# biiiipy/JaxMARL-HFT

Measured on AMD Instinct MI355X. Metric: env steps/sec (whole node), 2-agent MARL, 10-level LOB, NUM_ENVS=4096, higher is better.
Workload: dtype int32

## Files before the change

### jaxmarl-hft_amd/csrc/hftlob.hip

```cpp
#include <hip/hip_runtime.h>
#include <stdint.h>
#include <string.h>
#include <stdio.h>
#include <mutex>
#include <type_traits>
#include <limits.h>

#include "../../include/hftlob.h"

typedef int32_t i32;
typedef uint32_t u32;
typedef uint8_t u8;
#define DEV __device__ __forceinline__

DEV int lane_id() { return __lane_id(); }
DEV i32 rdl(i32 v, int l) { return __builtin_amdgcn_readlane(v, l); }
DEV i32 wrl(i32 old, i32 val, int l) { return __lane_id() == l ? val : old; }
DEV i32 uni(i32 v) { return __builtin_amdgcn_readfirstlane(v); }
DEV float unif(float v) { return __int_as_float(__builtin_amdgcn_readfirstlane(__float_as_int(v))); }
DEV i32 wadd(i32 a, i32 b) { return (i32)((u32)a + (u32)b); }
DEV i32 wsub(i32 a, i32 b) { return (i32)((u32)a - (u32)b); }
DEV i32 wmul(i32 a, i32 b) { return (i32)((u32)a * (u32)b); }
DEV i32 iabs_(i32 a) { return a < 0 ? wsub(0, a) : a; }
DEV i32 isign(i32 a) { return (a > 0) - (a < 0); }
// ... 1514 lines not shown
    i32* st = rec + c.off_agents;
    int ag = 0;
    for (int t = 0; t < nTy; ++t) {
        const hftlob_agent_type_cfg& tc = c.types[t];
        i32 sell = tc.task == HFTLOB_TASK_SELL ? 1 : 0;
        if (tc.kind == HFTLOB_AGENT_EXE && tc.task == HFTLOB_TASK_RANDOM)
            sell = randint(split_key(key, nTy + 1, t, part), 0, 2, part);
        for (int i = 0; i < tc.n_agents; ++i, ++ag) {
            i32 s[13];
            if (tc.kind == HFTLOB_AGENT_MM) {
                s[0] = 0; s[1] = 0; s[2] = 0; s[3] = fbit(0.0f); s[4] = fbit(0.0f);
            } else {
                s[0] = fbit(mid); s[1] = tc.task_size; s[2] = 0; s[3] = sell; s[4] = fbit(mid / (float)c.tick_size);
                for (int k = 5; k < 13; ++k) s[k] = fbit(0.0f);
            }
            const int nw = agent_words(tc);
            i32 v = 0;
            for (int k = 0; k < 13; ++k) if (l == k) v = s[k];
            if (l < nw) st[l] = v;
            if (obs) write_obs<false>(c, tc, wv, s, obs + (size_t)ag * c.obs_stride, false, ftime);
            st += nw;
        }
    }
}

template <int S>
__global__ __launch_bounds__(64) void k_env_reset(hftlob_env_cfg c, int n_env, const u32* __restrict__ keys,
                                                  const i32* __restrict__ init_states, i32* __restrict__ state,
                                                  float* __restrict__ obs) {
    one_wave();
    const int e = blockIdx.x;
    if (e >= n_env) return;
    Valid<S> VS, VT;
    VS.init(c.lob.n_orders);
    VT.init(c.lob.n_trades);
    Key k{keys[2 * e], keys[2 * e + 1]};
    env_reset_dev<S>(c, k, init_states, state + (size_t)e * c.rec_words,
                     obs ? obs + (size_t)e * c.n_agents * c.obs_stride : nullptr, VS, VT, c.ep_type == 1);
}

struct ActX {
    i32 bid_price, ask_price, bid_dist, ask_dist, bid_quant, ask_quant;
};

DEV void put_row(i32* lds_rows, int row, i32 f0, i32 f1, i32 f2, i32 f3, i32 f4, i32 f5, i32 f6, i32 f7) {
    const int l = lane_id();
    i32 v = f0;
    v = l == 1 ? f1 : v; v = l == 2 ? f2 : v; v = l == 3 ? f3 : v;
    v = l == 4 ? f4 : v; v = l == 5 ? f5 : v; v = l == 6 ? f6 : v; v = l == 7 ? f7 : v;
    if (l < 8) lds_rows[row * 8 + l] = v;
}

template <int S>
DEV void cancel_rows(const Side<S>& s, int R, const Valid<S>& V, i32 agent, int size, i32 side, i32 t, i32 tns,
                     i32* lds_rows, int row0) {
    int n = 0;
    i32 tid[S], q[S], o[S];
    const i32 (&p)[S] = s.pc;
    ldcol(s.t, R, FTID, tid);
    ldcol(s.t, R, FQ, q);
    ldcol(s.t, R, FOID, o);
#pragma unroll
    for (int r = 0; r < S; ++r) {
        lmask bm = V.m[r] & bal(tid[r] == agent);
        while (bm && n < size) {
            const int ln = (int)__builtin_ctzll(bm);
            bm &= bm - 1;
            put_row(lds_rows, row0 + n, 2, side, rdl(q[r], ln), rdl(p[r], ln), rdl(o[r], ln), agent, t, tns);
            ++n;
        }
    }
    for (; n < size; ++n) put_row(lds_rows, row0 + n, 2, side, 0, 0, 0, 0, t, tns);
}

template <int n>
DEV void filter_rows(i32* lds_rows, int arow, int crow, i32* scratch) {
    wave_sync();
    const int l = lane_id();
    const bool is_a = l < n, is_c = (l >= 8) & (l < 8 + n);
    const int row = is_a ? arow + l : (is_c ? crow + l - 8 : arow);
    const i32 p = lds_rows[row * 8 + 3], q = lds_rows[row * 8 + 2];
    lmask ma = 0, mc = 0;
#pragma unroll
    for (int k = 0; k < n; ++k) {
        const i32 cpk = rdl(p, 8 + k), apk = rdl(p, k);
        ma |= bal(is_a & (p != 0) & (p == cpk));
        mc |= bal(is_c & (apk != 0) & (p == apk));
    }
    constexpr lmask amask = (1ull << n) - 1, cmask = amask << 8;
    const int na = __builtin_popcountll(ma), nc = __builtin_popcountll(mc);
    const lmask mine = is_a ? ma : mc, all = is_a ? amask : cmask;
    const bool matched = (mine >> l) & 1ull;
    const lmask below = matched ? mine : (~mine & all);
    const int cnt = (int)__builtin_amdgcn_mbcnt_hi((u32)(below >> 32), __builtin_amdgcn_mbcnt_lo((u32)below, 0u));
    const int rank = matched ? cnt : (is_a ? na : nc) + cnt;
    if (l < 16) scratch[l] = 0;
    wave_sync();
    if ((is_a | is_c) & matched) scratch[(is_c ? 8 : 0) + rank] = q;
    wave_sync();
    const i32 av = scratch[rank & 7], cv = scratch[8 + (rank & 7)];
    const i32 nq = wsub(q, cv >= av ? av : 0);
    if (is_a & (nq == 0)) {
        reinterpret_cast<int4*>(lds_rows + row * 8)[0] = make_int4(0, 0, 0, 0);
        reinterpret_cast<int4*>(lds_rows + row * 8)[1] = make_int4(0, 0, 0, 0);
    } else if (is_a | is_c) {
        lds_rows[row * 8 + 2] = nq;
    }
    wave_sync();
}

template <int S>
DEV bool masked_best(const hftlob_env_cfg& c, Book<S>& B, i32 tid, i32 last_ba, i32 last_bb, i32& ba, i32& bb) {
    const i32 tick = c.tick_size;
    i32 mn = INT_MAX, mx = INT_MIN, at_[S], bt_[S];
    const i32 (&ap_)[S] = B.a.pc;
    const i32 (&bp_)[S] = B.b.pc;
    ldcol(B.a.t, B.c.nO, FTID, at_);
    ldcol(B.b.t, B.c.nO, FTID, bt_);
#pragma unroll
    for (int r = 0; r < S; ++r) {
        const i32 pa = (B.vs.v[r] && at_[r] != tid) ? ap_[r] : -1;
        const i32 pb = (B.vs.v[r] && bt_[r] != tid) ? bp_[r] : -1;
        mn = imin_(mn, B.vs.v[r] ? (pa == -1 ? c.lob.maxint : pa) : INT_MAX);
        mx = imax_(mx, B.vs.v[r] ? pb : INT_MIN);
    }
    ba = wave_min(mn);
    bb = wave_max(mx);
    ba = ba == c.lob.maxint ? -1 : ba;
    const bool empty = (ba == -1) || (bb == -1);
    ba = wmul(tick_floordiv(c, ba), tick);
    bb = wmul(tick_floordiv(c, bb), tick);
    if (empty) { bb = last_bb; ba = last_ba; }
    return empty;
}
template <int S>
DEV void mm_fixed_quant(const hftlob_env_cfg& c, const hftlob_agent_type_cfg& tc, Book<S>& B, const i32* st, i32 tid,
                        i32 action, i32 wt0, i32 wt1, i32 last_ba, i32 last_bb, i32* lds_rows, int row, ActX& x) {
    if (tc.fixed_action_setting) action = tc.fixed_action;
    const i32 tick = c.tick_size;
    i32 ba, bb;
    const bool empty = masked_best(c, B, tid, last_ba, last_bb, ba, bb);
    const float hsp = fmaxf(i2f(wsub(ba, bb)) / 2.0f, (float)tick / 2.0f);
    const float hs = (tick_ffloordiv(c, hsp) + 1.0f) * (float)tick;
    float bo, ao;
    i32 bq, aq;
    if (!tc.sell_buy_all_option) {
        const int ai = action < 0 ? imax_(action + 10, 0) : (action > 9 ? 9 : action);
        bo = (float)((0x0152043210ull >> (4 * ai)) & 0xF);
        ao = (float)((0x0510243210ull >> (4 * ai)) & 0xF);
        const i32 q1 = ai == 9 ? 0 : 1;
        bq = wmul(q1, tc.fixed_quant_value);
        aq = wmul(q1, tc.fixed_quant_value);
    } else {
        const int ai = action < 0 ? imax_(action + 9, 0) : (action > 8 ? 8 : action);
        const i32 bot[9] = {10, 2, 4, -1, 0, 2, -20, 0, 0}, aot[9] = {10, 2, 4, -1, 2, 0, 0, -20, 0};
        const i32 iq = ifloordiv(st[2], tc.fixed_quant_value);
        i32 b = bot[0], a = aot[0];
#pragma unroll
        for (int k = 1; k < 9; ++k) { b = ai == k ? bot[k] : b; a = ai == k ? aot[k] : a; }
        bo = i2f(b);
        ao = i2f(a);
        bq = wmul(ai < 6 ? 1 : (ai == 6 ? iq : 0), tc.fixed_quant_value);
        aq = wmul(ai < 6 ? 1 : (ai == 7 ? iq : 0), tc.fixed_quant_value);
    }
    if (empty) { bq = 0; aq = 0; }
    const float bpf = i2f(bb) - bo * hs;
    const float apf = i2f(ba) + ao * hs;
    const i32 bp = f2i(tick_ffloordiv(c, fmaxf(bpf, 0.0f)) * (float)tick);
    const i32 ap = f2i(tick_ffloordiv(c, fmaxf(i2f(wadd(bp, tick)), apf)) * (float)tick);
    i32 typ0 = 1, typ1 = 1, sd0 = 1, sd1 = -1, qq0 = bq, qq1 = aq, pp0 = bp, pp1 = ap;
    const i32 inv = st[2];
    const i32 lq0 = f2i(tc.auto_liquidate_alpha * i2f(imax_(wsub(0, inv), 0)));
    const i32 lq1 = f2i(tc.auto_liquidate_alpha * i2f(imax_(inv, 0)));
    const i32 lp0 = f2i(i2f(ba) + hs * 10.0f), lp1 = f2i(i2f(bb) - hs * 10.0f);
    const bool liq = (tc.tenth_action_market && action == 9) ||
                     (tc.auto_liquidate_threshold != 0 && iabs_(inv) > tc.auto_liquidate_threshold);
    if (liq) { typ0 = typ1 = 4; sd0 = -1; sd1 = 1; qq0 = lq0; qq1 = lq1; pp0 = lp0; pp1 = lp1; }
    const i32 ta = wadd(wt0, tc.time_delay_obs_act), tb = wadd(wt1, tc.time_delay_obs_act);
    put_row(lds_rows, row, typ0, sd0, qq0, pp0, c.placeholder_order_id, tid, ta, tb);
    put_row(lds_rows, row + 1, typ1, sd1, qq1, pp1, c.placeholder_order_id, tid, ta, tb);
    x.bid_price = bp; x.ask_price = ap; x.bid_dist = wsub(bb, bp); x.ask_dist = wsub(ap, ba);
    x.bid_quant = bq; x.ask_quant = aq;
}

DEV i32 f2i_sat(float f) {
    return f != f ? 0 : (f >= 2147483648.0f ? INT_MAX : (f <= -2147483648.0f ? INT_MIN : (i32)f));
}
template <int S>
DEV void mm_other_actions(const hftlob_env_cfg& c, const hftlob_agent_type_cfg& tc, Book<S>& B, const i32* st, i32 tid,
                          i32 action, i32 wt0, i32 wt1, i32 last_ba, i32 last_bb, i32 step, i32 init_t0, i32* lds_rows,
                          int row, ActX& x) {
    if (tc.fixed_action_setting) action = tc.fixed_action;
    const i32 tick = c.tick_size, inv = st[2], fq = tc.fixed_quant_value;
    const int kind = tc.action_space;
    const int na = kind == HFTLOB_MM_ACT_SIMPLE ? (tc.simple_nothing_action ? 4 : 3)
                                                 : (kind == HFTLOB_MM_ACT_AVST ? 8 : 2 * tc.bob_v0 + 1);
    int ai = action < 0 ? action + na : action;
    ai = ai < 0 ? 0 : (ai >= na ? na - 1 : ai);
    i32 bp, ap, bq, aq, bdist = 0, adist = 0, bpost = 0, apost = 0;
    if (kind == HFTLOB_MM_ACT_BOB_RL || kind == HFTLOB_MM_ACT_BOB_STRATEGY || kind == HFTLOB_MM_ACT_AVST) {
        i32 ba, bb;
        const bool empty = masked_best(c, B, tid, last_ba, last_bb, ba, bb);
        if (kind == HFTLOB_MM_ACT_BOB_RL) {
            const i32 v0 = tc.bob_v0, d = (ai & 1) ? (ai + 1) / 2 : -(ai / 2);
            bq = wmul(wadd(v0, d), fq);
            aq = wmul(wsub(v0, d), fq);
            if (empty) { bq = 0; aq = 0; }
            bp = bb; ap = ba;
        } else if (kind == HFTLOB_MM_ACT_BOB_STRATEGY) {
            const float kappa = i2f(wadd(action, 1)) / i2f(wmul(tc.bob_v0, 5));
            const float pos = i2f(inv), v0 = (float)tc.bob_v0;
            bq = f2i_sat(rintf(v0 * fmaxf(1.0f - kappa * pos, 0.0f)));
            aq = f2i_sat(rintf(v0 * fmaxf(1.0f + kappa * pos, 0.0f)));
            if (empty) { bq = 0; aq = 0; }
            bp = bb; ap = ba;
        } else {
            const i32 mid = ifloordiv(wadd(ba, bb), 2);
            const float gam[8] = {0.1f, 0.2f, 0.5f, 1.0f, 2.0f, 5.0f, 10.0f, 20.0f};
            float gamma = gam[0], lt = tc.avst_log_term[0];
#pragma unroll
            for (int k = 1; k < 8; ++k) if (ai == k) { gamma = gam[k]; lt = tc.avst_log_term[k]; }
            const i32 tl = c.ep_type == 1 ? wsub(c.episode_time, wsub(wt0, init_t0)) : wsub(c.episode_time, step);
            const float nt = i2f(tl) / i2f(c.episode_time);
            const float res = i2f(mid) - i2f(inv) * gamma * tc.avst_var * nt;
            float spread = gamma * tc.avst_var * nt + (2.0f / gamma) * lt;
            spread = fminf(fmaxf(spread, (float)tick), (float)c.lob.maxint);
            float bf = res - spread / 2.0f, af = res + spread / 2.0f;
            bf = fminf(fmaxf(bf, 0.0f), (float)c.lob.maxint);
            af = fminf(fmaxf(af, 0.0f), (float)c.lob.maxint);
            bp = f2i_sat(tick_ffloordiv(c, bf) * (float)tick);
            ap = f2i_sat(tick_ffloordiv(c, af) * (float)tick);
            const i32 q = tick_floordiv(c, mid), rm = wsub(mid, wmul(q, tick));
            bp = imin_(bp, wmul(wsub(q, rm == 0 ? 1 : 0), tick));
            ap = imax_(ap, wmul(wadd(q, 1), tick));
            bq = fq; aq = fq;
            bdist = wsub(bb, bp); adist = wsub(ap, ba); bpost = bp; apost = ap;
        }
    } else {
        const i32 ba = wmul(tick_floordiv(c, last_ba), tick), bb = wmul(tick_floordiv(c, last_bb), tick);
        if (kind == HFTLOB_MM_ACT_SPREAD_SKEW) {
            const float mid = i2f(wadd(ba, bb)) / 2.0f;
            const i32 cur = wsub(ba, bb);
            const i32 st_ = ifloordiv(action, 3), sk = wsub(action, wmul(st_, 3));
            const float mult = st_ == 0 ? 1.0f : tc.spread_multiplier;
            const float nsp = i2f(cur) * mult;
            const float skt = sk == 0 ? -tc.skew_multiplier : (sk == 1 ? 0.0f : tc.skew_multiplier);
            const float smid = mid + skt * (tc.multiplier_type ? nsp : (float)tick);
            const float hs = ffloordiv(nsp, 2.0f);
            bp = f2i_sat(tick_ffloordiv(c, smid - hs) * (float)tick);
            ap = f2i_sat(tick_ffloordiv(c, smid + hs) * (float)tick);
            bq = fq; aq = fq;
        } else {
            const float bo = ai == 1 ? -2000.0f : 0.0f, ao = ai == 2 ? -2000.0f : 0.0f;
            if (tc.sell_buy_all_option) {
                const i32 big = imax_(iabs_(inv), fq);
                const i32 bqa = inv > 0 ? fq : big, aqa = inv > 0 ? big : fq;
                bq = ai == 0 ? fq : (ai == 1 ? bqa : 0);
                aq = ai == 0 ? fq : (ai == 2 ? aqa : 0);
            } else {
                bq = wmul((ai == 0 || ai == 1) ? 1 : 0, fq);
                aq = wmul((ai == 0 || ai == 2) ? 1 : 0, fq);
            }
            const float to = (float)wmul(tc.n_ticks_offset, tick);
            const float bf = i2f(bb) - bo * to, af = i2f(ba) + ao * to;
            bp = f2i_sat(tick_ffloordiv(c, fmaxf(bf, 0.0f)) * (float)tick);
            ap = f2i_sat(tick_ffloordiv(c, af) * (float)tick);
        }
    }
    const i32 ta = wadd(wt0, tc.time_delay_obs_act), tb = wadd(wt1, tc.time_delay_obs_act);
    put_row(lds_rows, row, 1, 1, bq, bp, c.placeholder_order_id, tid, ta, tb);
    put_row(lds_rows, row + 1, 1, -1, aq, ap, c.placeholder_order_id, tid, ta, tb);
    x.bid_price = bpost; x.ask_price = apost; x.bid_dist = bdist; x.ask_dist = adist;
    x.bid_quant = bq; x.ask_quant = aq;
}

DEV void mm_directional(const hftlob_env_cfg& c, const hftlob_agent_type_cfg& tc, i32 tid, i32 action, i32 wt0, i32 wt1,
                        i32 last_ba, i32 last_bb, i32* lds_rows, int row, ActX& x) {
    const i32 tick = c.tick_size;
    const i32 ba = wmul(tick_floordiv(c, last_ba), tick), bb = wmul(tick_floordiv(c, last_bb), tick);
    const int ai = action < 0 ? imax_(action + 3, 0) : (action > 2 ? 2 : action);
    const i32 bq = (ai == 1) * tc.fixed_quant_value, aq = (ai == 2) * tc.fixed_quant_value;
    const i32 ta = wadd(wt0, tc.time_delay_obs_act), tb = wadd(wt1, tc.time_delay_obs_act);
    put_row(lds_rows, row, 1, 1, bq, ba, c.placeholder_order_id, tid, ta, tb);
    put_row(lds_rows, row + 1, 1, -1, aq, bb, c.placeholder_order_id, tid, ta, tb);
    x.bid_price = x.ask_price = x.bid_dist = x.ask_dist = 0;
    x.bid_quant = bq; x.ask_quant = aq;
}

DEV void exe_fqc(const hftlob_env_cfg& c, const hftlob_agent_type_cfg& tc, const i32* st, i32 tid, i32 action, i32 wt0,
                 i32 wt1, i32 last_ba, i32 last_bb, i32 step, i32 max_steps, i32* lds_rows, int row) {
    const i32 tick = c.tick_size;
    const i32 ba = wmul(tick_floordiv(c, last_ba), tick), bb = wmul(tick_floordiv(c, last_bb), tick);
    const i32 sell = st[3];
    i32 pl[4];
    if (sell) {
        pl[0] = bb;
        pl[1] = f2i(ceilf(tick_ffloordiv(c, i2f(wadd(bb, ba)) / 2.0f)) * (float)tick);
        pl[2] = ba;
        pl[3] = wadd(ba, wmul(tick, tc.n_ticks_in_book));
    } else {
        pl[0] = ba;
        pl[1] = wmul(tick_floordiv(c, ifloordiv(wadd(bb, ba), 2)), tick);
        pl[2] = bb;
        pl[3] = wsub(bb, wmul(tick, tc.n_ticks_in_book));
    }
    const i32 side = wsub(1, wmul(sell, 2));
    const i32 ta = wadd(wt0, tc.time_delay_obs_act), tb = wadd(wt1, tc.time_delay_obs_act);
    const i32 fq = tc.fixed_quant_value, left = wsub(st[1], st[2]);
    i32 q[4] = {0, 0, 0, 0};
    if (tc.action_space == HFTLOB_EXE_ACT_FIXED_QUANTS_COMPLEX) {
        const int ai = action < 0 ? imax_(action + 13, 0) : (action > 12 ? 12 : action);
        if (ai > 0) {
            const int lvl = (ai - 1) & 3, mul = (ai - 1) >> 2;
            const i32 v = wmul(mul == 0 ? 1 : (mul == 1 ? 2 : 5), fq);
#pragma unroll
            for (int k = 0; k < 4; ++k) q[k] = k == lvl ? v : 0;
        }
        const i32 tot = wadd(wadd(q[0], q[1]), wadd(q[2], q[3]));
        if (!(tot <= left)) { q[0] = f2i(floorf(i2f(left))); q[1] = q[2] = q[3] = 0; }
        for (int k = 0; k < 4; ++k) put_row(lds_rows, row + k, 1, side, q[k], pl[k], c.placeholder_order_id, tid, ta, tb);
        return;
    }
    if (tc.action_space == HFTLOB_EXE_ACT_FIXED_QUANTS_1MSG) {
        const int ai = action < 0 ? imax_(action + 5, 0) : (action > 4 ? 4 : action);
        i32 p = 0;
#pragma unroll
        for (int k = 0; k < 4; ++k) p = ai == k + 1 ? pl[k] : p;
        i32 qq = ai == 0 ? 0 : fq;
        qq = qq <= left ? qq : 0;
        put_row(lds_rows, row, 1, side, qq, p, c.placeholder_order_id, tid, ta, tb);
        return;
    }
    const i32 ft = sell ? bb : ba, nt = sell ? ba : bb;
    if (tc.action_space == HFTLOB_EXE_ACT_SIMPLEST_CASE) {
        const int ai = action < 0 ? imax_(action + 3, 0) : (action > 2 ? 2 : action);
        q[0] = ai == 1 ? fq : 0;
        q[1] = ai == 2 ? fq : 0;
        if (!(wadd(q[0], q[1]) <= left)) { q[0] = f2i(floorf(i2f(wmul(fq, left)))); q[1] = 0; }
    } else {
        const int ai = action < 0 ? imax_(action + 2, 0) : (action > 1 ? 1 : action);
        const i32 steps_left = wsub(wsub(max_steps, step), 1);
        const i32 qts = f2i_sat(ceilf(i2f(imax_(left, 0)) / i2f(steps_left)));
        q[0] = ai == 0 ? qts : 0;
        q[1] = ai == 1 ? qts : 0;
    }
    put_row(lds_rows, row, 1, side, q[0], ft, c.placeholder_order_id, tid, ta, tb);
    put_row(lds_rows, row + 1, 1, side, q[1], nt, c.placeholder_order_id, tid, ta, tb);
}

DEV void exe_fixed_prices(const hftlob_env_cfg& c, const hftlob_agent_type_cfg& tc, const i32* rec, const i32* st,
                          i32 tid, const i32 (&act)[4], i32 wt0, i32 wt1, i32* lds_rows, int row) {
    const i32 tick = c.tick_size, w = tc.n_actions, left = wsub(st[1], st[2]), sell = st[3];
    i32 sum = 0;
    for (int j = 0; j < w; ++j) sum = wadd(sum, act[j]);
    i32 q[4];
    const bool rescale = sum > left;
    for (int j = 0; j < 4; ++j) q[j] = rescale ? f2i_sat(i2f(act[j]) / i2f(sum) * i2f(left)) : act[j];
    const int M = c.n_msgs, m0 = M > 10 ? M - 10 : 0;
    float sa = 0.0f, sb = 0.0f;
    for (int m = m0; m < M; ++m) {
        sa += i2f(rec[c.off_best_asks + m * 2]);
        sb += i2f(rec[c.off_best_bids + m * 2]);
    }
    const float n = (float)(M - m0), ft = (float)tick;
    const i32 ba = f2i_sat(ffloordiv(sa / n, ft) * ft), bb = f2i_sat(ffloordiv(sb / n, ft) * ft);
    i32 lv[4];
    if (sell) {
        lv[0] = wmul(tick_floordiv(c, bb), tick);
        lv[1] = f2i_sat(ceilf(ffloordiv(i2f(wadd(bb, ba)) / 2.0f, ft)) * ft);
        lv[2] = ba;
        lv[3] = wadd(ba, wmul(tick, tc.n_ticks_in_book));
    } else {
        lv[0] = wmul(tick_floordiv(c, ba), tick);
        lv[1] = wmul(tick_floordiv(c, ifloordiv(wadd(bb, ba), 2)), tick);
        lv[2] = bb;
        lv[3] = wsub(bb, wmul(tick, tc.n_ticks_in_book));
    }
    i32 p[4];
    if (w == 4) { p[0] = lv[0]; p[1] = lv[1]; p[2] = lv[2]; p[3] = lv[3]; }
    else { p[0] = lv[0]; p[1] = lv[2]; p[2] = lv[3]; p[3] = 0; }
    if (w == 4 && lv[1] == lv[2]) {
        q[2] = wadd(q[2], q[1]);
        q[1] = 0;
        p[1] = -1;
    }
    const i32 side = wsub(1, wmul(sell, 2));
    const i32 ta = wadd(wt0, tc.time_delay_obs_act), tb = wadd(wt1, tc.time_delay_obs_act);
    for (int j = 0; j < w; ++j) put_row(lds_rows, row + j, 1, side, q[j], p[j], c.placeholder_order_id, tid, ta, tb);
}

template <int S>
struct TradeView {
    i32 P[S], Q[S], S4[S], PT[S], AT[S];
    bool valid[S];
};
template <int S>
DEV void trade_view(const Book<S>& B, TradeView<S>& V, bool use_ovr, int ovr_idx, const i32 (&ovr)[8]) {
    const int l = lane_id();
#pragma unroll
    for (int r = 0; r < S; ++r) {
        const bool o = use_ovr && (r * 64 + l == ovr_idx);
        const i32 p = o ? ovr[0] : B.tr.get(0, r), q = o ? ovr[1] : B.tr.get(1, r);
        const i32 s4 = o ? ovr[4] : B.tr.get(4, r), pt = o ? ovr[6] : B.tr.get(6, r), at = o ? ovr[7] : B.tr.get(7, r);
        const bool v = B.vt.v[r] && p >= 0;
// ... 739 lines not shown
    const StepKeys SK = batched ? load_keys(c, pre_keys) : step_keys<NFIX == 0>(c, key_n, ek, keys, master, mk);
    if (master && !batched) mk = SK.next_master;
    const Key key_reset = SK.key_reset;
    if (RC) {
        B.ek = c.shuffle_action_messages ? split_key(SK.k1, 2, 0, c.prng_partitionable) : SK.k1;
        B.nmsg = M;
        B.part = c.prng_partitionable;
    }
    SUBSTAMP(t_keys);
    const i32* Lr = rec + c.off_loaded;
    const i32* Wr = rec + c.off_world;
    const i32 ld_t0 = Lr[LD_T0], win = Lr[LD_WIN], max_steps = Lr[LD_MAXS], start_index = Lr[LD_START],
              step = Lr[LD_STEP];
    const i32 wt0 = Wr[W_T0], wt1 = Wr[W_T1], oidc = Wr[W_OIDC];
    const float wmid = bitf(Wr[W_MID]);
    const i32 old_last_ba = rec[c.off_best_asks + (M - 1) * 2], old_last_bb = rec[c.off_best_bids + (M - 1) * 2];
    bool excl_any = false, excl_cfg = false;
    for (int t = 0; t < c.n_types; ++t) {
        const bool ex = c.types[t].kind == HFTLOB_AGENT_MM && c.types[t].exclude_extreme_spreads;
        excl_cfg |= ex;
        if (emit && ex) {
            bool any = false;
            for (int m = l; m < M; m += 64) {
                const i32 pa = rec[c.off_best_asks + m * 2], pb = rec[c.off_best_bids + m * 2];
                any |= (i2f(wsub(pa, pb)) / (i2f(wadd(pa, pb)) / 2.0f)) > 0.1f;
            }
            excl_any = ballot(any) != 0ull;
        }
    }
    const bool store_best = NFIX == 0 || (!keep | excl_cfg);
    i32 dstart = wadd(start_index, wmul(D, step));
    dstart = imax_(0, imin_(dstart, c.n_data_rows - D));
    const bool ftime = NFIX == 0 && c.ep_type == 1;
    const i32 t_end = wadd(ld_t0, c.episode_time);
    int4 px = make_int4(0, 0, 0, 0), py = px;
    if ((l >= C + A) & (l < M)) {
        const i32* g = msg_data + (size_t)(dstart + l - (C + A)) * 8;
        ld_msg(g, px, py);
        if (ftime) fixed_time_mask(px, py, t_end);
    }
    if (resident) {
        relink_side(B.a, R, B.vs);
        relink_side(B.b, R, B.vs);
        B.fl = fl_carry | F_STALE_A | F_STALE_B | STALE_ANY;
    } else {
        B.fl = commit_side<true>(B.a, fa, R, B.vs) | commit_side<false>(B.b, fb, R, B.vs) | F_STALE_A | F_STALE_B | STALE_ANY;
        B.fl |= slow_bit(B.fl);
    }
    SUBSTAMP(t_load);

#ifdef HFTLOB_STAMPS
    unsigned long long acc_act = 0, acc_cnl = 0, acc_flt = 0, acc_mmr = 0, acc_exr = 0, acc_obs = 0;
#endif
    {
        int ag = 0, arow = C, crow = 0, aw = 0;
        const i32* st = rec + c.off_agents;
        for (int t = 0; t < c.n_types; ++t) {
            const hftlob_agent_type_cfg& tc = c.types[t];
            for (int i = 0; i < tc.n_agents; ++i, ++ag) {
                const i32 tid = wsub(tc.trader_id0, i);
                const int w = tc.action_width;
                i32* aio = actions_io ? actions_io + (size_t)e * c.action_words + aw : nullptr;
                aw += w;
                i32 act, av[4] = {0, 0, 0, 0};
                if (NFIX > 0 || w == 1) {
                    if (master) {
                        act = rdl(SK.acts, 32 + ag);
                        if (aio && l == 0) aio[0] = act;
                    } else {
                        act = aio[0];
                    }
                    av[0] = act;
                } else {
                    i32 v = 0;
                    if (master) {
                        const bool part = c.prng_partitionable;
                        const Key ka = split_key(split_key(SK.key, c.n_types, t, part), tc.n_agents, i, part);
                        v = randint_vec(ka, w, l < w ? l : 0, 0, action_hi(tc), part);
                        if (aio && l < w) aio[l] = v;
                    } else if (l < w) {
                        v = aio[l];
                    }
#pragma unroll
                    for (int j = 0; j < 4; ++j) av[j] = rdl(v, j);
                    act = av[0];
                }
                i32 s4[4];
                {
                    const int b = (int)(st - (rec + c.off_agents));
#pragma unroll
                    for (int k = 0; k < 4; ++k) s4[k] = agw_pre ? rdl(agw, b + k) : st[k];
                }
                ActX x{0, 0, 0, 0, 0, 0};
                SUBSTAMP(ta0);
#if defined(HFTLOB_KO_ACT) || defined(HFTLOB_KO_CNL)
                for (int k = 0; k < tc.n_msgs; ++k) {
#ifndef HFTLOB_KO_ACT
                    if (k < tc.n_action_msgs) continue;
#endif
#ifndef HFTLOB_KO_CNL
                    if (k >= tc.n_action_msgs) continue;
#endif
                    put_row(rows, k < tc.n_action_msgs ? arow + k : crow + k - tc.n_action_msgs, 0, 0, 0, 0, 0, 0, 0, 0);
                }
#endif
#ifdef HFTLOB_DUP_AGENT
                i32 z_ = 0;
                asm volatile("s_mov_b32 %0, 0" : "=s"(z_));
                for (int rep = 0; rep < 2; ++rep) {
                const i32 tid_r = tid ^ (rep * z_), act_r = act ^ (rep * z_), ba_r = old_last_ba ^ (rep * z_);
                const bool do_act = rep == 0 || (HFTLOB_DUP_AGENT & 1), do_cnl = rep == 0 || (HFTLOB_DUP_AGENT & 2);
#else
                {
                const i32 tid_r = tid, act_r = act, ba_r = old_last_ba;
                constexpr bool do_act = true, do_cnl = true;
#endif
                if (tc.kind == HFTLOB_AGENT_MM) {
#ifndef HFTLOB_KO_ACT
                    if (!do_act) {
                    } else if (tc.action_space == HFTLOB_MM_ACT_DIRECTIONAL)
                        mm_directional(c, tc, tid_r, act_r, wt0, wt1, ba_r, old_last_bb, rows, arow, x);
                    else if (tc.action_space == HFTLOB_MM_ACT_FIXED_QUANTS)
                        mm_fixed_quant(c, tc, B, s4, tid_r, act_r, wt0, wt1, ba_r, old_last_bb, rows, arow, x);
                    else
                        mm_other_actions(c, tc, B, s4, tid_r, act_r, wt0, wt1, ba_r, old_last_bb, step, ld_t0, rows,
                                         arow, x);
#endif
                    STAMP_ACC(acc_act, ta0);
                    SUBSTAMP(ta1);
                    const int sz = tc.n_msgs / 4;
#ifndef HFTLOB_KO_CNL
                    if (do_cnl) {
                        cancel_rows(B.b, R, B.vs, tid_r, sz, 1, wt0, wt1, rows, crow);
                        cancel_rows(B.a, R, B.vs, tid_r, sz, -1, wt0, wt1, rows, crow + sz);
                    }
#endif
                    STAMP_ACC(acc_cnl, ta1);
                } else {
#ifndef HFTLOB_KO_ACT
                    if (!do_act) {
                    } else if (NFIX == 0 && tc.action_space == HFTLOB_EXE_ACT_FIXED_PRICES)
                        exe_fixed_prices(c, tc, rec, s4, tid_r, av, wt0, wt1, rows, arow);
                    else
                        exe_fqc(c, tc, s4, tid_r, act_r, wt0, wt1, ba_r, old_last_bb, step, max_steps, rows, arow);
#endif
                    STAMP_ACC(acc_act, ta0);
                    SUBSTAMP(ta1);
#ifndef HFTLOB_KO_CNL
                    const i32 sell = s4[3];
                    if (do_cnl)
                        cancel_rows(sell ? B.a : B.b, R, B.vs, tid_r, tc.n_msgs / 2, wsub(1, wmul(sell, 2)), wt0, wt1,
                                    rows, crow);
#endif
                    STAMP_ACC(acc_cnl, ta1);
                }
                }
                SUBSTAMP(ta2);
                {
                    const i32 xv[6] = {x.bid_price, x.ask_price, x.bid_dist, x.ask_dist, x.bid_quant, x.ask_quant};
                    i32 v = 0;
#pragma unroll
                    for (int k = 0; k < 6; ++k) if (l == k) v = xv[k];
                    if (l < 6) axs[ag * 6 + l] = v;
                }
#ifndef HFTLOB_KO_FILTER
                if (tc.n_action_msgs == 2) filter_rows<2>(rows, arow, crow, B.a.scr);
                else if (tc.n_action_msgs == 4) filter_rows<4>(rows, arow, crow, B.a.scr);
                else if (NFIX == 0 && tc.n_action_msgs == 3) filter_rows<3>(rows, arow, crow, B.a.scr);
                else filter_rows<1>(rows, arow, crow, B.a.scr);
#endif
                STAMP_ACC(acc_flt, ta2);
                arow += tc.n_action_msgs;
                crow += tc.n_msgs - tc.n_action_msgs;
                st += agent_words(tc);
            }
        }
    }
    wave_sync();
    SUBSTAMP(t_rows);
    {
        i32 f[8];
        const bool act_lane = l < A;
        if (act_lane) {
#pragma unroll
            for (int k = 0; k < 8; ++k) f[k] = rows[(C + l) * 8 + k];
            f[4] = wsub(oidc, l);
        }
        int dest = l;
        if (c.shuffle_action_messages && A >= 2) {
            const u32 bits = SK.shuffle_bits;
            int rank = 0;
            for (int j = 0; j < A; ++j) {
                const u32 bj = (u32)rdl((i32)bits, j);
                rank += (bj < bits) || (bj == bits && j < l);
            }
            dest = rank;
        }
        wave_sync();
        if (act_lane) {
#pragma unroll
            for (int k = 0; k < 8; ++k) rows[(C + dest) * 8 + k] = f[k];
        }
        wave_sync();
    }

    STAMP(t_agents);
    if (!RA) trades_fill(B.tr, B.vt, -1);
    B.ntr = 0;
    const int AR = C + A;
    bool abort_any = false;
    i32 prev_a = -1, prev_b = -1;
    float mid_acc = 0.0f, pa_acc = 0.0f, pb_acc = 0.0f;
    i32 last_p_a = 0, last_p_b = 0, last_t0 = 0, last_t1 = 0;
    int4 nx = px, ny = py;
#ifndef HFTLOB_NO_CARRY
    i32* carry = B.filt - PAD_FILT + PAD_CARRY;
    if (!RA && resident) {
        const i32 v = carry[l & 15];
        B.a.best_p = rdl(v, 0); B.a.best_q = rdl(v, 1); B.a.xp = rdl(v, 2); B.a.top = rdl(v, 3);
        B.a.top_p = rdl(v, 4); B.a.top_ts = rdl(v, 5); B.a.top_tns = rdl(v, 6);
        B.b.best_p = rdl(v, 7); B.b.best_q = rdl(v, 8); B.b.top = rdl(v, 9); B.b.top_p = rdl(v, 10);
        B.b.top_ts = rdl(v, 11); B.b.top_tns = rdl(v, 12);
        B.fl &= ~(F_STALE_A | F_STALE_B | STALE_ANY);
    }
#endif
#ifdef HFTLOB_STAMPS_CHUNK
    unsigned long long acc_dec = 0, acc_pre = 0, acc_loop = 0, acc_post = 0;
#endif
    for (int base = 0; base < M; base += 64) {
#ifdef HFTLOB_STAMPS_CHUNK
        const unsigned long long tc0 = __builtin_amdgcn_s_memtime();
#endif
        const int row = base + l;
        int4 x = nx, y = ny;
        if (RA ? (base == 0) & (row < AR) : row < AR) {
            x = reinterpret_cast<const int4*>(rows + row * 8)[0];
            y = reinterpret_cast<const int4*>(rows + row * 8)[1];
        } else if (ftime && base > 0 && row >= AR) {
            fixed_time_mask(x, y, t_end);
        }
        if (msgs_out && row < M) {
            int4* mo = reinterpret_cast<int4*>(msgs_out + ((size_t)e * M + row) * 8);
            mo[0] = x;
            mo[1] = y;
        }
        {
            const bool nv = (row + 64 >= AR) & (row + 64 < M);
            ld_msg(msg_data + (size_t)(dstart + (nv ? row + 64 - AR : 0)) * 8, nx, ny);
        }
        if (RA && (base == 0)) {
            if (row + 64 < AR) {
                nx = reinterpret_cast<const int4*>(rows + (row + 64) * 8)[0];
                ny = reinterpret_cast<const int4*>(rows + (row + 64) * 8)[1];
            }
            wave_sync();
            trades_fill(B.tr, B.vt, -1);
        }
        decode_msgs(B.c, x, y);
        i32 rpa = 0, rqa = 0, rpb = 0, rqb = 0;
        const int cnt = uni(imin_(64, M - base));
#ifdef HFTLOB_STAMPS_CHUNK
        acc_dec += __builtin_amdgcn_s_memtime() - tc0;
#endif
        run_chunk<RC>(B, x, y, cnt, base, rpa, rqa, rpb, rqb CHUNK_ARGS);
#ifdef HFTLOB_STAMPS_CHUNK
        const unsigned long long tc1 = __builtin_amdgcn_s_memtime();
#endif
        abort_any |= bal((l < cnt) & ((rpa == -1) | (rpb == -1))) != 0ull;
        i32 pa = rpa, pb = rpb;
        if ((base == 0) & (l == 0)) {
            pa = pa == -1 ? old_last_ba : pa;
            pb = pb == -1 ? old_last_bb : pb;
        }
        const i32 caq = rpa == -1 ? 0 : rqa, cbq = rpb == -1 ? 0 : rqb;
        const i32 cap = ffill(pa, prev_a), cbp = ffill(pb, prev_b);
        prev_a = rdl(cap, cnt - 1);
        prev_b = rdl(cbp, cnt - 1);
        if ((row < M) & (store_best | (row == M - 1))) {
            reinterpret_cast<int2*>(rec + c.off_best_asks)[row] = make_int2(cap, caq);
            reinterpret_cast<int2*>(rec + c.off_best_bids)[row] = make_int2(cbp, cbq);
        }
        if (row < M) {
            const float mf = i2f(wadd(cbp, cap)) / 2.0f;
            mid_acc = base == 0 ? mf : mid_acc + mf;
            if (info_out) {
                pa_acc = base == 0 ? i2f(cap) : pa_acc + i2f(cap);
                pb_acc = base == 0 ? i2f(cbp) : pb_acc + i2f(cbp);
            }
// ... 643 lines not shown
                return fail(HFTLOB_EINVAL, "EXE action_width");
            if (tc.n_action_msgs != na || tc.n_msgs != 2 * na) return fail(HFTLOB_EINVAL, "EXE message counts");
            if (a == HFTLOB_EXE_ACT_TWAP && c->ep_type != 0) return fail(HFTLOB_EINVAL, "twap needs fixed_steps");
            if (tc.observation_space < 0 || tc.observation_space > HFTLOB_EXE_OBS_SIMPLEST_CASE)
                return fail(HFTLOB_EINVAL, "EXE observation_space");
        } else return fail(HFTLOB_EINVAL, "unknown agent kind");
    }
    if (agents != c->n_agents) return fail(HFTLOB_EINVAL, "n_agents mismatch");
    int words = 0;
    for (int t = 0; t < c->n_types; ++t) words += c->types[t].n_agents * c->types[t].action_width;
    if (words != c->action_words) return fail(HFTLOB_EINVAL, "action_words mismatch");
    return HFTLOB_OK;
}

static hftlob_env_cfg kernel_cfg(const hftlob_env_cfg* cfg) {
    hftlob_env_cfg c = *cfg;
    const uint32_t d = (uint32_t)c.tick_size;
    const int l = d > 1u ? 32 - __builtin_clz(d - 1u) : 0;
    c.tick_magic = (uint32_t)((((unsigned __int128)1 << (31 + l)) + d - 1u) / d);
    return c;
}

int hftlob_env_reset(const hftlob_env_cfg* cfg, int n_env, const uint32_t* keys, const int32_t* msg_data,
                     const int32_t* init_states, int32_t* state, const hftlob_step_out* out, void* stream) {
    int rc = check_env(cfg);
    if (rc) return rc;
    (void)msg_data;
    if (n_env < 0) return fail(HFTLOB_ESHAPE, "negative n_env");
    if (n_env == 0) return HFTLOB_OK;
    if (!keys || !init_states || !state) return fail(HFTLOB_ENULL, "null array");
    float* obs = out ? out->obs : nullptr;
    const int S = slot_sets(cfg->lob.n_orders > cfg->lob.n_trades ? cfg->lob.n_orders : cfg->lob.n_trades);
    hipStream_t st = (hipStream_t)stream;
    dim3 g(n_env), b(ENV_BLOCK);
    const hftlob_env_cfg kc = kernel_cfg(cfg);
    if (S == 1) hipLaunchKernelGGL(k_env_reset<1>, g, b, 0, st, kc, n_env, keys, init_states, state, obs);
    else if (S == 2) hipLaunchKernelGGL(k_env_reset<2>, g, b, 0, st, kc, n_env, keys, init_states, state, obs);
    else hipLaunchKernelGGL(k_env_reset<4>, g, b, 0, st, kc, n_env, keys, init_states, state, obs);
    return launch_status();
}

#ifndef HFTLOB_LDS_FLOOR
#define HFTLOB_LDS_FLOOR 0
#endif
static bool nfix_kernel(const hftlob_env_cfg* cfg) {
    return cfg->lob.cancel_mode < 2 && cfg->lob.n_orders == 100 && cfg->lob.n_trades == 100 && cfg->ep_type == 0 &&
           !has_fixed_prices(cfg);
}
static bool use_rows_alias(const hftlob_env_cfg* cfg) {
    return nfix_kernel(cfg) && rows_in_trades(*cfg, cfg->lob.n_trades) &&
           4 * lds_map(*cfg, cfg->lob.n_orders, cfg->lob.n_trades, false).words > 160 * 1024 / 16;
}

struct Variant {
    int S, nfix;
    bool rc, ra, kb;
};
static Variant env_variant(const hftlob_env_cfg* cfg) {
    Variant v;
    v.rc = cfg->lob.cancel_mode >= 2;
    v.nfix = nfix_kernel(cfg) ? 100 : 0;
    v.S = v.nfix ? 2 : slot_sets(cfg->lob.n_orders > cfg->lob.n_trades ? cfg->lob.n_orders : cfg->lob.n_trades);
    v.ra = use_rows_alias(cfg);
    v.kb = kb_ok(*cfg);
    return v;
}
extern "C++" {
template <int S_, int NFIX_, bool RC_, bool RA_> struct VariantT {
    static constexpr int S = S_, NFIX = NFIX_;
    static constexpr bool RC = RC_, RA = RA_;
};
template <class F> static bool with_variant(const Variant& v, F&& f) {
#define HFTLOB_X(SS, NF, RC, RA) \
    if (v.S == SS && v.nfix == NF && v.rc == RC && v.ra == RA) return f(VariantT<SS, NF, RC, RA>{}), true;
    HFTLOB_VARIANTS(HFTLOB_X)
#undef HFTLOB_X
    return false;
}
static size_t env_shm(const hftlob_env_cfg* cfg, const Variant& v) {
    const size_t b = 4 * (size_t)lds_map(*cfg, cfg->lob.n_orders, cfg->lob.n_trades, v.ra).words;
    return b < (size_t)HFTLOB_LDS_FLOOR ? (size_t)HFTLOB_LDS_FLOOR : b;
}
template <class Kernel, class... Args>
static int env_launch(const hftlob_env_cfg* cfg, int n_env, void* stream, Kernel&& kernel, Args... args) {
    const Variant v = env_variant(cfg);
    const hftlob_env_cfg kc = kernel_cfg(cfg);
    const bool listed = with_variant(v, [&](auto V) {
        hipLaunchKernelGGL(kernel(V, v), dim3(n_env), dim3(ENV_BLOCK), env_shm(cfg, v), (hipStream_t)stream, kc, n_env,
                           args...);
    });
    return listed ? launch_status() : fail(HFTLOB_ELAUNCH, "no kernel for the config's variant");
}
}

static int env_step_launch(const hftlob_env_cfg* cfg, int n_env, int key_e0, int key_n, const uint32_t* keys,
                           const uint32_t* key_in, uint32_t* key_out, int32_t* actions, const int32_t* msg_data,
                           const int32_t* init_states, int32_t* state, const hftlob_step_out* out, void* stream) {
    if (!out->obs || !out->rewards || !out->done_all || !out->dones) return fail(HFTLOB_ENULL, "null output");
    return env_launch(
        cfg, n_env, stream,
        [](auto V, const Variant&) { return k_env_step<decltype(V)::S, decltype(V)::NFIX, decltype(V)::RC, decltype(V)::RA>; },
        key_e0, key_n, keys, key_in, key_out, actions, msg_data, init_states, state, *out);
}

static int env_rollout_launch(const hftlob_env_cfg* cfg, int n_env, int key_e0, int key_n, int n_steps, int per_step,
                              const uint32_t* key_in, uint32_t* key_out, int32_t* actions, const int32_t* msg_data,
                              const int32_t* init_states, int32_t* state, const hftlob_step_out* out, void* stream) {
    return env_launch(
        cfg, n_env, stream,
        [](auto V, const Variant& v) {
            using T = decltype(V);
            if constexpr (T::NFIX > 0 && !T::RA)
                return v.kb ? k_env_rollout<T::S, T::NFIX, T::RC, T::RA, 1> : k_env_rollout<T::S, T::NFIX, T::RC, T::RA, 0>;
            else
                return k_env_rollout<T::S, T::NFIX, T::RC, T::RA, -1>;
        },
// ... 205 lines not shown
```

Before: 91.65 million.

## Keep agent action/cancel message rows in registers instead of LDS staging

For the fixed-size (NFIX) variant without the rows alias, agent action and cancel message rows are now built in per-lane registers (one row per lane), not written to and read back from LDS. The duplicate-price filter and the action shuffle are redone with ds_permute/bpermute cross-lane ops, and the order-book columns are loaded once and reused by masked_best and the cancels. This removes the LDS stores, wave syncs and reloads in the per-step message assembly. In exchange it adds register pressure and restricts the variant to configs with at most 64 agent messages.

```diff
diff --git a/jaxmarl-hft_amd/csrc/hftlob.hip b/jaxmarl-hft_amd/csrc/hftlob.hip
--- a/jaxmarl-hft_amd/csrc/hftlob.hip
+++ b/jaxmarl-hft_amd/csrc/hftlob.hip
@@ -1590,6 +1590,62 @@
 }
 
 template <int S>
+struct RegRows {
+    int4 x, y;
+    i32 meta;
+    i32 at[S], aq[S], ao[S], bt[S], bq[S], bo[S];
+    DEV void init(const i32* ta, const i32* tb, int R, int C, i32 t, i32 tns) {
+        const int l = lane_id();
+        const bool cl = l < C;
+        x = make_int4(cl ? 2 : 0, 0, 0, 0);
+        y = make_int4(0, 0, cl ? t : 0, cl ? tns : 0);
+        meta = l | l << 8;
+        ldcol(ta, R, FTID, at); ldcol(ta, R, FQ, aq); ldcol(ta, R, FOID, ao);
+        ldcol(tb, R, FTID, bt); ldcol(tb, R, FQ, bq); ldcol(tb, R, FOID, bo);
+    }
+    DEV void put(int row, i32 f0, i32 f1, i32 f2, i32 f3, i32, i32, i32, i32) {
+        const bool m = lane_id() == row;
+        x.x = m ? f0 : x.x; x.y = m ? f1 : x.y; x.z = m ? f2 : x.z; x.w = m ? f3 : x.w;
+    }
+    DEV void agent(int arow, int crow, int n, i32 tid, i32 t, i32 tns) {
+        const int l = lane_id();
+        const bool ia = (u32)(l - arow) < (u32)n, ic = (u32)(l - crow) < (u32)n;
+        y.y = ia ? tid : y.y; y.z = ia ? t : y.z; y.w = ia ? tns : y.w;
+        const i32 ma = arow | crow << 8 | (n - 1) << 16, mc = crow | arow << 8 | (n - 1) << 16;
+        meta = ia ? ma : (ic ? mc : meta);
+    }
+};
+template <int S>
+DEV void put_row(RegRows<S>* r, int row, i32 f0, i32 f1, i32 f2, i32 f3, i32 f4, i32 f5, i32 f6, i32 f7) {
+    r->put(row, f0, f1, f2, f3, f4, f5, f6, f7);
+}
+template <class T> struct is_reg_rows { static constexpr bool value = false; };
+template <int S> struct is_reg_rows<RegRows<S>*> { static constexpr bool value = true; };
+template <bool REG, int S> DEV auto row_sink(RegRows<S>& regs, i32* lds_rows) {
+    if constexpr (REG) return &regs;
+    else return lds_rows;
+}
+template <int S>
+DEV void cancel_regs(RegRows<S>& sink, const i32 (&tid)[S], const i32 (&q)[S], const i32 (&o)[S], const i32 (&p)[S],
+                     const Valid<S>& V, i32 agent, int size, i32 side, int row0) {
+    const int l = lane_id();
+    sink.x.y = (u32)(l - row0) < (u32)size ? side : sink.x.y;
+    int n = 0;
+#pragma unroll
+    for (int r = 0; r < S; ++r) {
+        lmask bm = V.m[r] & bal(tid[r] == agent);
+        while (bm && n < size) {
+            const int ln = (int)__builtin_ctzll(bm);
+            bm &= bm - 1;
+            const bool m = l == row0 + n;
+            sink.x.z = m ? rdl(q[r], ln) : sink.x.z; sink.x.w = m ? rdl(p[r], ln) : sink.x.w;
+            sink.y.x = m ? rdl(o[r], ln) : sink.y.x; sink.y.y = m ? agent : sink.y.y;
+            ++n;
+        }
+    }
+}
+
+template <int S>
 DEV void cancel_rows(const Side<S>& s, int R, const Valid<S>& V, i32 agent, int size, i32 side, i32 t, i32 tns,
                      i32* lds_rows, int row0) {
     int n = 0;
@@ -1646,15 +1702,46 @@
     }
     wave_sync();
 }
-
 template <int S>
-DEV bool masked_best(const hftlob_env_cfg& c, Book<S>& B, i32 tid, i32 last_ba, i32 last_bb, i32& ba, i32& bb) {
+DEV void filter_regs(RegRows<S>& s, int C) {
+    const int l = lane_id();
+    const int own = s.meta & 0xFF, oth = (s.meta >> 8) & 0xFF, g1 = s.meta >> 16, off = l - own;
+    const i32 p = s.x.w, q = s.x.z;
+    bool hit = false;
+#pragma unroll
+    for (int r = 0; r < 4; ++r) hit |= __builtin_amdgcn_ds_bpermute((oth + ((off + r) & g1)) << 2, p) == p;
+    const bool matched = hit & (p != 0);
+    const lmask M = bal(matched);
+    const u32 grp = (u32)(M >> own) & ((2u << g1) - 1u);
+    const int mb = __builtin_popcount(grp & ((1u << off) - 1u));
+    const int rank = matched ? mb : __builtin_popcount(grp) + off - mb;
+    const bool is_a = l >= C;
+    const int slot = ((is_a ? own : oth) + rank) << 2;
+    const i32 av = __builtin_amdgcn_ds_permute((matched & is_a) ? slot : 0, q);
+    const i32 cv = __builtin_amdgcn_ds_permute((matched & !is_a) ? slot : 0, q);
+    const i32 nq = wsub(q, __builtin_amdgcn_ds_bpermute(slot, cv >= av ? av : 0));
+    if (is_a & (nq == 0)) {
+        s.x = make_int4(0, 0, 0, 0);
+        s.y = s.x;
+    } else {
+        s.x.z = nq;
+    }
+}
+
+template <int S, class Rows>
+DEV bool masked_best(const hftlob_env_cfg& c, Book<S>& B, const Rows lds_rows, i32 tid, i32 last_ba, i32 last_bb, i32& ba,
+                     i32& bb) {
     const i32 tick = c.tick_size;
     i32 mn = INT_MAX, mx = INT_MIN, at_[S], bt_[S];
     const i32 (&ap_)[S] = B.a.pc;
     const i32 (&bp_)[S] = B.b.pc;
-    ldcol(B.a.t, B.c.nO, FTID, at_);
-    ldcol(B.b.t, B.c.nO, FTID, bt_);
+    if constexpr (is_reg_rows<Rows>::value) {
+#pragma unroll
+        for (int r = 0; r < S; ++r) { at_[r] = lds_rows->at[r]; bt_[r] = lds_rows->bt[r]; }
+    } else {
+        ldcol(B.a.t, B.c.nO, FTID, at_);
+        ldcol(B.b.t, B.c.nO, FTID, bt_);
+    }
 #pragma unroll
     for (int r = 0; r < S; ++r) {
         const i32 pa = (B.vs.v[r] && at_[r] != tid) ? ap_[r] : -1;
@@ -1671,13 +1758,13 @@
     if (empty) { bb = last_bb; ba = last_ba; }
     return empty;
 }
-template <int S>
+template <int S, class Rows>
 DEV void mm_fixed_quant(const hftlob_env_cfg& c, const hftlob_agent_type_cfg& tc, Book<S>& B, const i32* st, i32 tid,
-                        i32 action, i32 wt0, i32 wt1, i32 last_ba, i32 last_bb, i32* lds_rows, int row, ActX& x) {
+                        i32 action, i32 wt0, i32 wt1, i32 last_ba, i32 last_bb, Rows lds_rows, int row, ActX& x) {
     if (tc.fixed_action_setting) action = tc.fixed_action;
     const i32 tick = c.tick_size;
     i32 ba, bb;
-    const bool empty = masked_best(c, B, tid, last_ba, last_bb, ba, bb);
+    const bool empty = masked_best(c, B, lds_rows, tid, last_ba, last_bb, ba, bb);
     const float hsp = fmaxf(i2f(wsub(ba, bb)) / 2.0f, (float)tick / 2.0f);
     const float hs = (tick_ffloordiv(c, hsp) + 1.0f) * (float)tick;
     float bo, ao;
@@ -1724,9 +1811,9 @@
 DEV i32 f2i_sat(float f) {
     return f != f ? 0 : (f >= 2147483648.0f ? INT_MAX : (f <= -2147483648.0f ? INT_MIN : (i32)f));
 }
-template <int S>
+template <int S, class Rows>
 DEV void mm_other_actions(const hftlob_env_cfg& c, const hftlob_agent_type_cfg& tc, Book<S>& B, const i32* st, i32 tid,
-                          i32 action, i32 wt0, i32 wt1, i32 last_ba, i32 last_bb, i32 step, i32 init_t0, i32* lds_rows,
+                          i32 action, i32 wt0, i32 wt1, i32 last_ba, i32 last_bb, i32 step, i32 init_t0, Rows lds_rows,
                           int row, ActX& x) {
     if (tc.fixed_action_setting) action = tc.fixed_action;
     const i32 tick = c.tick_size, inv = st[2], fq = tc.fixed_quant_value;
@@ -1738,7 +1825,7 @@
     i32 bp, ap, bq, aq, bdist = 0, adist = 0, bpost = 0, apost = 0;
     if (kind == HFTLOB_MM_ACT_BOB_RL || kind == HFTLOB_MM_ACT_BOB_STRATEGY || kind == HFTLOB_MM_ACT_AVST) {
         i32 ba, bb;
-        const bool empty = masked_best(c, B, tid, last_ba, last_bb, ba, bb);
+        const bool empty = masked_best(c, B, lds_rows, tid, last_ba, last_bb, ba, bb);
         if (kind == HFTLOB_MM_ACT_BOB_RL) {
             const i32 v0 = tc.bob_v0, d = (ai & 1) ? (ai + 1) / 2 : -(ai / 2);
             bq = wmul(wadd(v0, d), fq);
@@ -1812,8 +1899,9 @@
     x.bid_quant = bq; x.ask_quant = aq;
 }
 
+template <class Rows>
 DEV void mm_directional(const hftlob_env_cfg& c, const hftlob_agent_type_cfg& tc, i32 tid, i32 action, i32 wt0, i32 wt1,
-                        i32 last_ba, i32 last_bb, i32* lds_rows, int row, ActX& x) {
+                        i32 last_ba, i32 last_bb, Rows lds_rows, int row, ActX& x) {
     const i32 tick = c.tick_size;
     const i32 ba = wmul(tick_floordiv(c, last_ba), tick), bb = wmul(tick_floordiv(c, last_bb), tick);
     const int ai = action < 0 ? imax_(action + 3, 0) : (action > 2 ? 2 : action);
@@ -1825,8 +1913,9 @@
     x.bid_quant = bq; x.ask_quant = aq;
 }
 
+template <class Rows>
 DEV void exe_fqc(const hftlob_env_cfg& c, const hftlob_agent_type_cfg& tc, const i32* st, i32 tid, i32 action, i32 wt0,
-                 i32 wt1, i32 last_ba, i32 last_bb, i32 step, i32 max_steps, i32* lds_rows, int row) {
+                 i32 wt1, i32 last_ba, i32 last_bb, i32 step, i32 max_steps, Rows lds_rows, int row) {
     const i32 tick = c.tick_size;
     const i32 ba = wmul(tick_floordiv(c, last_ba), tick), bb = wmul(tick_floordiv(c, last_bb), tick);
     const i32 sell = st[3];
@@ -1886,8 +1975,9 @@
     put_row(lds_rows, row + 1, 1, side, q[1], nt, c.placeholder_order_id, tid, ta, tb);
 }
 
+template <class Rows>
 DEV void exe_fixed_prices(const hftlob_env_cfg& c, const hftlob_agent_type_cfg& tc, const i32* rec, const i32* st,
-                          i32 tid, const i32 (&act)[4], i32 wt0, i32 wt1, i32* lds_rows, int row) {
+                          i32 tid, const i32 (&act)[4], i32 wt0, i32 wt1, Rows lds_rows, int row) {
     const i32 tick = c.tick_size, w = tc.n_actions, left = wsub(st[1], st[2]), sell = st[3];
     i32 sum = 0;
     for (int j = 0; j < w; ++j) sum = wadd(sum, act[j]);
@@ -2733,6 +2823,14 @@
 #ifdef HFTLOB_STAMPS
     unsigned long long acc_act = 0, acc_cnl = 0, acc_flt = 0, acc_mmr = 0, acc_exr = 0, acc_obs = 0;
 #endif
+    constexpr bool REG = NFIX > 0 && !RA;
+    RegRows<S> sink;
+    if constexpr (REG) {
+        SUBSTAMP(tc0);
+        sink.init(B.a.t, B.b.t, R, C, wt0, wt1);
+        STAMP_ACC(acc_cnl, tc0);
+    }
+    const auto srows = row_sink<REG>(sink, rows);
     {
         int ag = 0, arow = C, crow = 0, aw = 0;
         const i32* st = rec + c.off_agents;
@@ -2782,7 +2880,7 @@
 #ifndef HFTLOB_KO_CNL
                     if (k >= tc.n_action_msgs) continue;
 #endif
-                    put_row(rows, k < tc.n_action_msgs ? arow + k : crow + k - tc.n_action_msgs, 0, 0, 0, 0, 0, 0, 0, 0);
+                    put_row(srows, k < tc.n_action_msgs ? arow + k : crow + k - tc.n_action_msgs, 0, 0, 0, 0, 0, 0, 0, 0);
                 }
 #endif
 #ifdef HFTLOB_DUP_AGENT
@@ -2800,18 +2898,23 @@
 #ifndef HFTLOB_KO_ACT
                     if (!do_act) {
                     } else if (tc.action_space == HFTLOB_MM_ACT_DIRECTIONAL)
-                        mm_directional(c, tc, tid_r, act_r, wt0, wt1, ba_r, old_last_bb, rows, arow, x);
+                        mm_directional(c, tc, tid_r, act_r, wt0, wt1, ba_r, old_last_bb, srows, arow, x);
                     else if (tc.action_space == HFTLOB_MM_ACT_FIXED_QUANTS)
-                        mm_fixed_quant(c, tc, B, s4, tid_r, act_r, wt0, wt1, ba_r, old_last_bb, rows, arow, x);
+                        mm_fixed_quant(c, tc, B, s4, tid_r, act_r, wt0, wt1, ba_r, old_last_bb, srows, arow, x);
                     else
-                        mm_other_actions(c, tc, B, s4, tid_r, act_r, wt0, wt1, ba_r, old_last_bb, step, ld_t0, rows,
+                        mm_other_actions(c, tc, B, s4, tid_r, act_r, wt0, wt1, ba_r, old_last_bb, step, ld_t0, srows,
                                          arow, x);
 #endif
                     STAMP_ACC(acc_act, ta0);
                     SUBSTAMP(ta1);
                     const int sz = tc.n_msgs / 4;
 #ifndef HFTLOB_KO_CNL
-                    if (do_cnl) {
+                    if constexpr (REG) {
+                        if (do_cnl) {
+                            cancel_regs(sink, sink.bt, sink.bq, sink.bo, B.b.pc, B.vs, tid_r, sz, 1, crow);
+                            cancel_regs(sink, sink.at, sink.aq, sink.ao, B.a.pc, B.vs, tid_r, sz, -1, crow + sz);
+                        }
+                    } else if (do_cnl) {
                         cancel_rows(B.b, R, B.vs, tid_r, sz, 1, wt0, wt1, rows, crow);
                         cancel_rows(B.a, R, B.vs, tid_r, sz, -1, wt0, wt1, rows, crow + sz);
                     }
@@ -2821,17 +2924,23 @@
 #ifndef HFTLOB_KO_ACT
                     if (!do_act) {
                     } else if (NFIX == 0 && tc.action_space == HFTLOB_EXE_ACT_FIXED_PRICES)
-                        exe_fixed_prices(c, tc, rec, s4, tid_r, av, wt0, wt1, rows, arow);
+                        exe_fixed_prices(c, tc, rec, s4, tid_r, av, wt0, wt1, srows, arow);
                     else
-                        exe_fqc(c, tc, s4, tid_r, act_r, wt0, wt1, ba_r, old_last_bb, step, max_steps, rows, arow);
+                        exe_fqc(c, tc, s4, tid_r, act_r, wt0, wt1, ba_r, old_last_bb, step, max_steps, srows, arow);
 #endif
                     STAMP_ACC(acc_act, ta0);
                     SUBSTAMP(ta1);
 #ifndef HFTLOB_KO_CNL
                     const i32 sell = s4[3];
-                    if (do_cnl)
+                    if constexpr (REG) {
+                        if (do_cnl) {
+                            if (sell) cancel_regs(sink, sink.at, sink.aq, sink.ao, B.a.pc, B.vs, tid_r, tc.n_msgs / 2, -1, crow);
+                            else cancel_regs(sink, sink.bt, sink.bq, sink.bo, B.b.pc, B.vs, tid_r, tc.n_msgs / 2, 1, crow);
+                        }
+                    } else if (do_cnl) {
                         cancel_rows(sell ? B.a : B.b, R, B.vs, tid_r, tc.n_msgs / 2, wsub(1, wmul(sell, 2)), wt0, wt1,
                                     rows, crow);
+                    }
 #endif
                     STAMP_ACC(acc_cnl, ta1);
                 }
@@ -2844,11 +2953,16 @@
                     for (int k = 0; k < 6; ++k) if (l == k) v = xv[k];
                     if (l < 6) axs[ag * 6 + l] = v;
                 }
+                if constexpr (REG)
+                    sink.agent(arow, crow, tc.n_action_msgs, tid, wadd(wt0, tc.time_delay_obs_act),
+                               wadd(wt1, tc.time_delay_obs_act));
 #ifndef HFTLOB_KO_FILTER
-                if (tc.n_action_msgs == 2) filter_rows<2>(rows, arow, crow, B.a.scr);
-                else if (tc.n_action_msgs == 4) filter_rows<4>(rows, arow, crow, B.a.scr);
-                else if (NFIX == 0 && tc.n_action_msgs == 3) filter_rows<3>(rows, arow, crow, B.a.scr);
-                else filter_rows<1>(rows, arow, crow, B.a.scr);
+                if constexpr (!REG) {
+                    if (tc.n_action_msgs == 2) filter_rows<2>(rows, arow, crow, B.a.scr);
+                    else if (tc.n_action_msgs == 4) filter_rows<4>(rows, arow, crow, B.a.scr);
+                    else if (NFIX == 0 && tc.n_action_msgs == 3) filter_rows<3>(rows, arow, crow, B.a.scr);
+                    else filter_rows<1>(rows, arow, crow, B.a.scr);
+                }
 #endif
                 STAMP_ACC(acc_flt, ta2);
                 arow += tc.n_action_msgs;
@@ -2857,9 +2971,33 @@
             }
         }
     }
+#ifndef HFTLOB_KO_FILTER
+    if constexpr (REG) {
+        SUBSTAMP(tf0);
+        filter_regs(sink, C);
+        STAMP_ACC(acc_flt, tf0);
+    }
+#endif
     wave_sync();
     SUBSTAMP(t_rows);
-    {
+    if constexpr (REG) {
+        const int j = l - C;
+        const bool act_lane = (j >= 0) & (j < A);
+        if (act_lane) sink.y.x = wsub(oidc, j);
+        if (c.shuffle_action_messages && A >= 2) {
+            const u32 bits = (u32)__builtin_amdgcn_ds_bpermute((j & 63) << 2, (i32)SK.shuffle_bits);
+            int rank = 0;
+            for (int k = 0; k < A; ++k) {
+                const u32 bk = (u32)rdl((i32)SK.shuffle_bits, k);
+                rank += (bk < bits) || (bk == bits && k < j);
+            }
+            const int dest = (act_lane ? C + rank : l) << 2;
+            sink.x.x = __builtin_amdgcn_ds_permute(dest, sink.x.x); sink.x.y = __builtin_amdgcn_ds_permute(dest, sink.x.y);
+            sink.x.z = __builtin_amdgcn_ds_permute(dest, sink.x.z); sink.x.w = __builtin_amdgcn_ds_permute(dest, sink.x.w);
+            sink.y.x = __builtin_amdgcn_ds_permute(dest, sink.y.x); sink.y.y = __builtin_amdgcn_ds_permute(dest, sink.y.y);
+            sink.y.z = __builtin_amdgcn_ds_permute(dest, sink.y.z); sink.y.w = __builtin_amdgcn_ds_permute(dest, sink.y.w);
+        }
+    } else {
         i32 f[8];
         const bool act_lane = l < A;
         if (act_lane) {
@@ -2894,6 +3032,9 @@
     float mid_acc = 0.0f, pa_acc = 0.0f, pb_acc = 0.0f;
     i32 last_p_a = 0, last_p_b = 0, last_t0 = 0, last_t1 = 0;
     int4 nx = px, ny = py;
+    if constexpr (REG) {
+        if (l < AR) { nx = sink.x; ny = sink.y; }
+    }
 #ifndef HFTLOB_NO_CARRY
     i32* carry = B.filt - PAD_FILT + PAD_CARRY;
     if (!RA && resident) {
@@ -2914,7 +3055,8 @@
 #endif
         const int row = base + l;
         int4 x = nx, y = ny;
-        if (RA ? (base == 0) & (row < AR) : row < AR) {
+        if (REG) {
+        } else if (RA ? (base == 0) & (row < AR) : row < AR) {
             x = reinterpret_cast<const int4*>(rows + row * 8)[0];
             y = reinterpret_cast<const int4*>(rows + row * 8)[1];
         } else if (ftime && base > 0 && row >= AR) {
@@ -3664,6 +3806,8 @@
            4 * lds_map(*cfg, cfg->lob.n_orders, cfg->lob.n_trades, false).words > 160 * 1024 / 16;
 }
 
+static bool reg_rows_ok(const hftlob_env_cfg* cfg) { return cfg->n_cancel_msgs + cfg->n_action_msgs <= 64; }
+
 struct Variant {
     int S, nfix;
     bool rc, ra, kb;
@@ -3671,9 +3815,9 @@
 static Variant env_variant(const hftlob_env_cfg* cfg) {
     Variant v;
     v.rc = cfg->lob.cancel_mode >= 2;
-    v.nfix = nfix_kernel(cfg) ? 100 : 0;
+    v.ra = use_rows_alias(cfg);
+    v.nfix = nfix_kernel(cfg) && (v.ra || reg_rows_ok(cfg)) ? 100 : 0;
     v.S = v.nfix ? 2 : slot_sets(cfg->lob.n_orders > cfg->lob.n_trades ? cfg->lob.n_orders : cfg->lob.n_trades);
-    v.ra = use_rows_alias(cfg);
     v.kb = kb_ok(*cfg);
     return v;
 }
```

After: 92.99 million (median of 6 runs). +1.5%, better.
